# shuaigroup/Renormalizer

Measured on AMD Instinct MI355X. Metric: TDVP-PS sweep site-updates/sec at (Nsite=50, Dbond=256, dphys=2/16), higher is better.
Workload: dtype c128

## Files before the change

### renormalizer_amd/csrc/mpse_contract.hip

```cpp
#include <deque>

#include "mpse_internal.h"
#include "mpse_plans.h"

using namespace mpse_plan;

namespace {

__device__ __forceinline__ long long off2(const mpse_index m, long long i) {
  if (m.lo_ext >= m.ext) return i * m.s_lo;
  const long long hi = i / m.lo_ext;
  return hi * m.s_hi + (i - hi * m.lo_ext) * m.s_lo;
}

template <typename T>
__global__ __launch_bounds__(256) void k_copy_strided(T* dst, const T* src, mpse_index mi, mpse_index ni, mpse_index mo,
                                                      mpse_index no, const int* skip) {
  if (skip && *skip) return;
  const long long nn = ni.ext;
  const long long total = mi.ext * nn;
  const long long stride = (long long)gridDim.x * blockDim.x;
  for (long long t = (long long)blockIdx.x * blockDim.x + threadIdx.x; t < total; t += stride) {
    const long long i = t / nn, j = t - i * nn;
    dst[off2(mo, i) + off2(no, j)] = src[off2(mi, i) + off2(ni, j)];
// ... 376 lines not shown
            o.seg[q].bm = fb + sg.bm_kt0;
          } else if (sg.bm_kind == BM_CENTRE && cm) {
            o.seg[q].bm = cm;
            gd.bm_pitch = cm_pitch;
          }
        }
      }
      gd.masks_stable = stable;
      if (gd.ngrp == 1 && s.groups[0].split2) {
        if (!bufs[B_OUT2]) return mpse_fail(ctx, MPSE_ERR_ARG, "plan: missing second result");
        gd.split2 = true;
        gd.c2 = const_cast<void*>(bufs[B_OUT2]);
      }
      const bool completes =
          &s == &p.steps.back() && gd.ngrp == 1 && s.groups[0].cbuf == B_OUT && s.groups[0].c_off == 0;
      MPSE_TRY(gemm_grouped(ctx, gd, sc, completes ? dot : nullptr));
      continue;
    }
    const char* a = (const char*)bufs[s.a] + size_t(s.a_off) * dtype_size(s.dta);
    const char* b = (const char*)bufs[s.b] + size_t(s.b_off) * dtype_size(s.dtb);
    const int dtc = (s.dta == MPSE_C128 || s.dtb == MPSE_C128) ? MPSE_C128 : MPSE_F64;
    if (dtc != dtype)
      return mpse_fail(ctx, MPSE_ERR_ARG, "plan step dtype mismatch (got %d want %d)", dtc, dtype);
    char* c = (char*)const_cast<void*>(bufs[s.c]) + size_t(s.c_off) * dtype_size(dtc);
    if (!bufs[s.a] || !bufs[s.b] || !bufs[s.c]) return mpse_fail(ctx, MPSE_ERR_ARG, "plan: missing buffer");
    if (s.kind == K_COPY) {
      MPSE_TRY(copy_call(ctx, dtc, a, c, s.ma, s.ka, s.mc, s.nc, skip));
      continue;
    }
    ProductReq rq;
    if (&s == &p.steps.back() && s.c == B_OUT && s.c_off == 0 && s.batch == 1) rq.dot = dot;
// ... 235 lines not shown
```

### renormalizer_amd/csrc/mpse_gemm.hip

```cpp
#include <cstdlib>

#include "mpse_device.h"
#include "mpse_internal.h"
#include "mpse_plans.h"

typedef double v4d __attribute__((ext_vector_type(4)));

static unsigned long long* gemm_trace_ptr(const mpse_ctx* ctx) {
  static const bool f0_only = [] {
    const char* e = getenv("MPSE_GEMM_TRACE_ONLY");
    return e && e[0] == 'f';
  }();
  return (ctx->prof_on && !f0_only) ? ctx->gemm_trace : nullptr;
}

namespace {

struct IdxMap {
  long long s_hi, s_lo;
  int ext, lo;
};

constexpr int GMAX_GRP = 8, GMAX_SEG = 4, GMAX_MIX = 8;
struct GMix {
// ... 10 lines not shown
  GSeg seg[GMAX_SEG];
  double* C;
  int nseg;
  int use_beta;
};
struct GemmGroups {
  GGrp g[GMAX_GRP];
  int ngrp, tiles_m_grp, nkt_seg, am_pitch, bm_pitch;
  int split2, cpd;
  double* C2;
  const unsigned long long* flags;
  int nmix, mix_grp, mix_d, mix_wr;
  long long mix_ld;
  const double* mix_w;
  GMix mix[GMAX_MIX];
};

struct GemmArgs {
  const double* A;
  const double* B;
  double* C;
  IdxMap mA, kA, kB, nB, mC, nC;
  long long sbA, sbB, sbC;
  int M, N, K;
  int tiles_m, tiles_n;
  int mtiles_m, mtiles_n;
  int a_kfast, b_kfast;
  int conjA, conjB;
  int use_beta;
  double alpha_re, alpha_im, beta_re, beta_im;
// ... 18 lines not shown
};


__device__ __forceinline__ void dot_acc(double& re, double& im, double2 c, double2 y) {
  re += c.x * y.x + c.y * y.y;
  im += c.x * y.y - c.y * y.x;
}

__device__ __forceinline__ long long idx_off(const IdxMap& m, int i) {
  if (m.lo == 0x7fffffff) return (long long)i * m.s_lo;
  const int hi = i / m.lo;
  const int l = i - hi * m.lo;
  return (long long)hi * m.s_hi + (long long)l * m.s_lo;
}

#ifndef MPSE_GEMM_3M
#define MPSE_GEMM_3M 1
#endif
constexpr int BM = 64, BN = 64, BK = 16, LDK = BK + 1;

template <bool CA, bool CB, bool KS, int WS, int WI = 2, bool GRP = false>
__global__ __launch_bounds__(64 * WS * WS * (2 / WI), WS == 1 ? 1 : WI == 1 ? 4 : ((CA && CB) ? 2 : 3)) void k_gemm(const GemmArgs g) {
  static_assert(!GRP || (KS && WS == 2), "grouped launches use the single-level 64 x 64 kernel");
  constexpr int TBM = 32 * WS, TBN = 32 * WS, NT = 64 * WS * WS * (2 / WI);
  static_assert(WI == 2 || (WI == 1 && WS == 2), "eight-wave form only for 64 x 64 tiles");
  constexpr int LD = WS == 2 ? 80 : 48;
  constexpr int NLD = TBM * BK / NT;
  constexpr bool CC = CA || CB;
  constexpr int EA = CA ? 2 : 1, EB = CB ? 2 : 1, EC = CC ? 2 : 1;
  __shared__ double smem[(2 + (CA ? 1 : 0) + (CB ? 1 : 0)) * BK * LD];
// ... 25 lines not shown
        half = q & 1;
        t = ((q >> 1) << 3) | (bid & 7);
      } else {
        half = bid & 1;
        t = bid >> 1;
      }
      bs = half;
    }
  }
  if (g.slice_fast) {
    t = bid / g.ksplit;
    bs = bid - t * g.ksplit;
  }
  const int b = bs / g.ksplit;
  const int ks_id = bs - b * g.ksplit;
  if (g.perm) t = g.perm[(ks_id & 1) ? ntile - 1 - t : t];
  int tm = t / g.tiles_n;
  int tn = t - tm * g.tiles_n;
  if (g.die_group == 1) {
    const int x = t & 7, j = t >> 3;
    tm = x + 8 * (j / g.tiles_n);
    tn = j % g.tiles_n;
  } else if (g.die_group == 2) {
    const int x = t & 7, j = t >> 3;
    tn = x + 8 * (j / g.tiles_m);
    tm = j % g.tiles_m;
  }
  if (g.skew && !g.perm && !g.die_group) tn = (tn + tm) % g.tiles_n;

  int grp = 0;
  if constexpr (GRP) {
    grp = tm / g.gg.tiles_m_grp;
    tm -= grp * g.gg.tiles_m_grp;
// ... 466 lines not shown
    for (int kk = 0; kk < BK / 4; ++kk) {
      const int cb = kk & 1;
      if (kk + 1 < BK / 4) read_frag(cb ^ 1, kk + 1);
      mfma_group(cb);
    }
  }
  }

  if (g.trace) tr3 = __builtin_readcyclecounter();
  struct TraceEnd {
    const GemmArgs& g;
    unsigned long long t0, rt0, &t1, &t2, &t3;
    int tid;
    int& ktd;
    __device__ ~TraceEnd() {
      if (g.trace && tid == 0) {
        const unsigned long long slot = atomicAdd(g.trace, 1ull);
        if (slot < GEMM_TRACE_CAP) {
          unsigned long long* r = g.trace + 1 + slot * GEMM_TRACE_WORDS;
          unsigned xcc = 0;
          r[0] = ((unsigned long long)gridDim.x << 32) | (unsigned long long)blockIdx.x;
          r[1] = ((unsigned long long)(CA ? 1 : 0) << 62) | ((unsigned long long)(CB ? 1 : 0) << 61) |
                 ((unsigned long long)g.ksplit << 40) | ((unsigned long long)(unsigned)g.K << 8) | xcc;
          const unsigned hw = __builtin_amdgcn_s_getreg((31 << 11) | 4), xc = __builtin_amdgcn_s_getreg((31 << 11) | 20);
          r[2] = (unsigned long long)(unsigned)ktd | ((unsigned long long)(((xc & 0xf) << 16) | (hw & 0xffff)) << 32);
          r[3] = t0;
          r[4] = t1;
          r[5] = t2;
          r[6] = t3;
          r[7] = __builtin_readcyclecounter();
          r[8] = rt0;
          r[9] = __builtin_amdgcn_s_memrealtime();
        }
      }
    }
  } trace_end{g, tr0, rt0, tr1, tr2, tr3, tid, kt_done};
  if (g.kt_counter && tid == 0 && kt_done) atomicAdd(g.kt_counter, (unsigned long long)kt_done);
  if constexpr (M3) {
#pragma unroll
    for (int i = 0; i < WI; ++i)
#pragma unroll
      for (int j = 0; j < 2; ++j) {
        acc_im[i][j] = acc_im[i][j] - acc_re[i][j] - acc_t2[i][j];
        acc_re[i][j] = acc_re[i][j] - acc_t2[i][j];
      }
  }
  if (g.ksplit > 1) {
    double* wsb = g.ws + (long long)bs * g.M * g.N * EC;
#pragma unroll
// ... 85 lines not shown
            const double* pin = g.Cin ? g.Cin + (idx_off(g.mCin, gi) + cinn) * EC : C + co * EC;
            if constexpr (CC)
              pre_c[i][j][r] = *reinterpret_cast<const double2*>(pin);
            else
              pre_c[i][j][r] = make_double2(*pin, 0.0);
          }
          if (need_y) {
            if constexpr (CC)
              pre_y[i][j][r] = reinterpret_cast<const double2*>(g.dot_y)[co];
            else
              pre_y[i][j][r] = make_double2(g.dot_y[co], 0.0);
          }
        }
    }
  }
#pragma unroll
  for (int j = 0; j < 2; ++j) {
    const int gj = tn * TBN + wn * 32 + j * 16 + (lane & 15);
    if (gj >= g.N) continue;
    const long long coffn = idx_off(g.nC, gj);
#pragma unroll
    for (int i = 0; i < WI; ++i) {
#pragma unroll
      for (int r = 0; r < 4; ++r) {
        const int gi = tm * TBM + wm * WROWS + i * 16 + (lane >> 4) + 4 * r;
        if (gi >= g.M) continue;
        const long long co = idx_off(g.mC, gi) + coffn;
        double* p = C + co * EC;
        const double xr = acc_re[i][j][r];
        if constexpr (CC) {
          const double xi = acc_im[i][j][r];
          double2 o;
          o.x = g.alpha_re * xr - g.alpha_im * xi;
          o.y = g.alpha_re * xi + g.alpha_im * xr;
// ... 9 lines not shown
          *reinterpret_cast<double2*>(p) = o;
          if (need_y) {
            if constexpr (PRE)
              dot_acc(dre, dim, o, pre_y[i][j][r]);
            else
              dot_acc(dre, dim, o, reinterpret_cast<const double2*>(g.dot_y)[co]);
          }
        } else {
          double o = g.alpha_re * xr;
          if (need_c) o += g.beta_re * (g.Cin ? g.Cin[idx_off(g.mCin, gi) + idx_off(g.nCin, gj)] : *p);
          *p = o;
          if (need_y) dre += o * g.dot_y[co];
        }
      }
    }
  }
  if constexpr (WS == 2) {
    if (g.dot_y) {
      __shared__ double s_dot[2 * (NT / 64)];
      dre = wave_sum(dre);
      dim = wave_sum(dim);
      if (lane == 0) {
        s_dot[2 * wave] = dre;
        s_dot[2 * wave + 1] = dim;
      }
      __syncthreads();
      dre = dim = 0.0;
#pragma unroll
      for (int w = 0; w < NT / 64; ++w) {
        dre += s_dot[2 * w];
// ... 20 lines not shown
          key[hi] = a;
        }
      }
      __syncthreads();
    }
}
__device__ __forceinline__ int pow2_at_least(int x) {
  int n = 2;
  while (n < x) n <<= 1;
  return n;
}
__global__ __launch_bounds__(1024) void k_tile_order(const unsigned long long* __restrict__ amask,
                                                       const unsigned long long* __restrict__ bmask, int nkw, int nkt,
                                                       int tiles_m, int tiles_n, int by_die, int* __restrict__ perm,
                                                       const int* __restrict__ skip, const GemmGroups gg,
                                                       unsigned char* __restrict__ flags_out, int flags_pitch) {
  if (skip && *skip) return;
  __shared__ unsigned key[2048], ckey[2048];
  __shared__ int colw[2048];
  __shared__ unsigned char die_of[2048];
  const int ntile = tiles_m * tiles_n, tid = threadIdx.x;
  const bool part = by_die && tiles_n % 8 == 0 && tiles_n <= 2048;
  for (int c = tid; c < 2048; c += 1024) colw[c] = 0;
  __syncthreads();
  for (int i = tid; i < 2048; i += 1024) {
    unsigned cnt = 0;
    if (i < ntile) {
      const int tm = i / tiles_n, tn = i - tm * tiles_n;
      if (gg.ngrp > 0) {
        const int grp = tm / gg.tiles_m_grp, tml = tm - grp * gg.tiles_m_grp;
        const GGrp& G = gg.g[grp];
        for (int q = 0; q < G.nseg; ++q)
          for (int l = 0; l < gg.nkt_seg; ++l) {
            unsigned v = 1;
            if (G.seg[q].am) v &= G.seg[q].am[(long long)tml * gg.am_pitch + l];
            if (G.seg[q].bm) v &= G.seg[q].bm[(long long)tn * gg.bm_pitch + l];
            cnt += v;
            if (flags_out) flags_out[(long long)i * flags_pitch + q * gg.nkt_seg + l] = (unsigned char)v;
          }
        if (flags_out)
          for (int l = G.nseg * gg.nkt_seg; l < flags_pitch; ++l) flags_out[(long long)i * flags_pitch + l] = 0;
      } else {
        for (int w = 0; w < nkw; ++w) {
          unsigned long long x = 0x0101010101010101ull;
          if (amask) x &= amask[(long long)tm * nkw + w];
          if (bmask) x &= bmask[(long long)tn * nkw + w];
          const int valid = nkt - 8 * w;
          if (valid < 8) x &= (1ull << (8 * valid)) - 1ull;
          cnt += __popcll(x);
// ... 15 lines not shown
    __syncthreads();
  }
  for (int i = tid; i < 2048; i += 1024) {
    unsigned k = 0;
    if (i < ntile) {
      const unsigned die = part ? die_of[i % tiles_n] : 0u;
      k = (die << 28) | (key[i] << 16) | (unsigned)(0xFFFF - i);
    }
    key[i] = k;
  }
  __syncthreads();
  bitonic_desc(key, tid, pow2_at_least(ntile));
  const int per_die = ntile / 8;
  for (int i = tid; i < ntile; i += 1024) {
    const int s = part ? (7 - (i & 7)) * per_die + (i >> 3) : i;
    perm[i] = 0xFFFF - (int)(key[s] & 0xFFFFu);
  }
}

template <bool CC>
__global__ __launch_bounds__(256) void k_splitk_reduce(const GemmArgs g, int batch) {
  constexpr int EC = CC ? 2 : 1;
  if (g.skip && *g.skip) return;
  const long long mn = (long long)g.M * g.N;
  const int rows = g.M * batch;
  double dre = 0.0, dim = 0.0;
  for (int row = blockIdx.y; row < rows; row += gridDim.y) {
    const int b = row / g.M;
    const int i = row - b * g.M;
    const double* wrow = g.ws + ((long long)b * g.ksplit * mn + (long long)i * g.N) * EC;
    double* crow = g.C + ((long long)b * g.sbC + idx_off(g.mC, i)) * EC;
// ... 408 lines not shown
      const dim3 og((p.nkt + 3) / 4, oa.tiles > ob.tiles ? oa.tiles : ob.tiles, (unsigned)(2 * d->batch));
      hipLaunchKernelGGL(k_tile_occ, og, dim3(256), 0, ctx->stream, oa, ob, g.K, g.nkw, (int)d->batch, g.skip);
    }
    g.amask = static_cast<const unsigned long long*>(ma.mask);
    g.bmask = static_cast<const unsigned long long*>(mb.mask);
  }

  if (p.order) {
    SolveScope* const keep = sc && sc->keeps_env_masks && ma.stable && mb.stable ? sc : nullptr;
    int* pp = nullptr;
    bool sort = false;
    MPSE_TRY(perm_source(ctx, keep, {g.amask, g.bmask, g.tiles_m, g.tiles_n, p.nkt, nullptr},
                         size_t(g.tiles_m) * g.tiles_n * sizeof(int), PERM, &pp, &sort));
    if (sort)
      hipLaunchKernelGGL(k_tile_order, dim3(1), dim3(1024), 0, ctx->stream, g.amask, g.bmask, g.nkw, p.nkt, g.tiles_m,
                         g.tiles_n, 1, pp, g.skip, GemmGroups(), (unsigned char*)nullptr, 0);
    g.perm = pp;
  }

  count_paths(ctx->gemm_paths, p, d->batch > 1);
  const bool reduce = g.ksplit > 1 && !p.leave_slices;
  launch_gemm(ctx, g, p.nwg, ca, cb, p.fast, p.wide, false, reduce ? dim3((unsigned)p.rgx, (unsigned)p.rgy) : dim3(0),
              (int)d->batch);
  if (prof_this) prof_end(ctx, rec);
  MPSE_HIP(ctx, hipGetLastError());
  return MPSE_OK;
}

int occ_mask_get(mpse_ctx* ctx, SolveScope* sc, const void* ptr, int dtype, mpse_index r, mpse_index k,
                 TmpBuf& tmp, const unsigned char** flags, int* pitch, bool* stable) {
  IdxMap rm, km;
// ... 6 lines not shown
  MPSE_TRY(occ_mask_source(ctx, keep, key, nullptr, tmp.p, &m));
  if (m.scan) {
    const OccOperand oa = occ_operand(key, rm, km, fastest(km) <= fastest(rm), m);
    OccOperand ob = oa;
    ob.tiles = 0;
    hipLaunchKernelGGL(k_tile_occ, dim3(((key.K + BK - 1) / BK + 3) / 4, key.tiles, 2), dim3(256), 0, ctx->stream, oa, ob,
                       key.K, key.nkw, 1, sc ? sc->skip : nullptr);
    MPSE_HIP(ctx, hipGetLastError());
  }
  *flags = static_cast<const unsigned char*>(m.mask);
  *pitch = key.nkw * 8;
  *stable = m.stable;
  return MPSE_OK;
}

static double mix_sources(const GroupedDesc& d) {
  int n = 0;
  for (int t = 0; t < d.nmix; ++t) {
    bool seen = false;
    for (int u = 0; u < t; ++u) seen = seen || d.mix[u].src == d.mix[t].src;
    n += seen ? 0 : 1;
  }
  return n > 1 ? double(n - 1) : 0.0;
}

int gemm_grouped(mpse_ctx* ctx, const GroupedDesc& d, SolveScope* sc, MatvecReq::Dot* dot) {
  GemmArgs g = {};
  if (d.ngrp < 1 || d.ngrp > GMAX_GRP) return mpse_fail(ctx, MPSE_ERR_ARG, "grouped product: 1 .. %d groups", GMAX_GRP);
  if (!fill_maps(g, d.ma, d.ka, d.kb, d.nb, d.mc, d.nc))
    return mpse_fail(ctx, MPSE_ERR_SHAPE, "grouped product: extent out of range");
  if (g.M != g.mC.ext || g.N != g.nC.ext || g.K != g.kB.ext) return mpse_fail(ctx, MPSE_ERR_SHAPE, "grouped product: extents disagree");
  if (g.M == 0 || g.N == 0) return MPSE_OK;
  const bool ca = d.dta == MPSE_C128, cb = d.dtb == MPSE_C128;
  if (!is_single(g.kA) || !is_single(g.kB) || !fast_ok(g, ca, cb) || g.K % BK != 0 || g.K < BK ||
      (d.ngrp > 1 && g.M % BM != 0) || !cb)
    return mpse_fail(ctx, MPSE_ERR_SHAPE, "grouped product: needs single-level K indices, K a multiple of %d, group "
                     "heights a multiple of %d and a complex second operand", BK, BM);
  if (d.split2 && (d.ngrp != 1 || !d.c2 || g.M % BM != 0))
    return mpse_fail(ctx, MPSE_ERR_ARG, "grouped product: halved tiles need one group, whole tile rows and a second result");
  g.alpha_re = 1.0, g.beta_re = 1.0;
  g.ksplit = 1;
// ... 29 lines not shown
  g.use_beta = any_beta;
  if (d.nmix > 0) {
    if (!ca || d.nmix > GMAX_MIX || d.mix_grp < 0 || d.mix_grp >= d.ngrp || d.grp[d.mix_grp].beta != 1.0 || !d.mix_w ||
        d.mix_d < 1 || BM % d.mix_d != 0 || g.M % BM != 0 || d.mix_wr < 1 || d.mix_ld < g.N)
      return mpse_fail(ctx, MPSE_ERR_ARG, "grouped product: bad epilogue mix");
    gg.nmix = d.nmix, gg.mix_grp = d.mix_grp, gg.mix_d = d.mix_d, gg.mix_wr = d.mix_wr, gg.mix_ld = d.mix_ld;
    gg.mix_w = static_cast<const double*>(d.mix_w);
    for (int t = 0; t < d.nmix; ++t) {
      if (!d.mix[t].src || d.mix[t].delta <= -d.mix_d || d.mix[t].delta >= d.mix_d)
        return mpse_fail(ctx, MPSE_ERR_ARG, "grouped product: bad epilogue mix term");
      gg.mix[t] = GMix{static_cast<const double*>(d.mix[t].src), d.mix[t].b, d.mix[t].f, d.mix[t].delta, 0};
    }
  }

  const int nkt_max = max_seg * gg.nkt_seg;
  const mpse_plan::GroupedPlan p = mpse_plan::grouped_plan(g.M, g.N, d.ngrp, nkt_max, any_mask, d.split2, ca, n_cu_of(ctx));
  const long long ntile = (long long)p.tiles_m * p.tiles_n;
  if (ntile > 0x7fffffffLL) return mpse_fail(ctx, MPSE_ERR_SHAPE, "grouped product: grid too large");
  g.tiles_m = p.tiles_m;
  g.nkw = p.nkw;
  g.die_group = p.die_group;
  if (dot && d.ngrp == 1 && p.nwg >= 1 && p.nwg <= dot->cap) {
    g.dot_y = static_cast<const double*>(dot->y);
    g.dot_part = dot->part;
    dot->nb_out = (int)p.nwg;
  }
  mpse_ctx::ProfRec rec;
  const int variant = (ca ? 1 : 0) + (cb ? 2 : 0);
  const double mnk = double(g.M) * double(g.N) * double(g.K) * segs;
  const bool prof_this = prof_begin(ctx, variant, mnk * ((ca && cb) ? 8.0 : 4.0),
                                    segs * (double(g.M) * g.K * (ca ? 16 : 8) + double(g.K) * g.N * 16.0) +
                                        double(d.ngrp) * double(g.M) * g.N * 16.0 * (any_beta ? 2 : 1) +
                                        mix_sources(d) * double(g.M) * g.N * 16.0,
                                    &rec);
  g.kt_counter = prof_this && ctx->prof_ktiles ? ctx->prof_ktiles + variant : nullptr;

  TmpBuf PERM(ctx);
  if (p.order) {
    const size_t perm_bytes = (size_t(ntile) * sizeof(int) + 7) & ~size_t(7), flag_pitch = size_t(g.nkw) * 8;
    int* pp = nullptr;
    bool sort = false;
    MPSE_TRY(perm_source(ctx, sc && sc->keeps_env_masks && d.masks_stable ? sc : nullptr,
                         {gg.g[0].seg[0].am, gg.g[0].seg[0].bm, g.tiles_m, g.tiles_n, nkt_max + 1000 * d.ngrp, nullptr},
                         perm_bytes + size_t(ntile) * flag_pitch, PERM, &pp, &sort));
    if (sort)
      hipLaunchKernelGGL(k_tile_order, dim3(1), dim3(1024), 0, ctx->stream, (const unsigned long long*)nullptr,
                         (const unsigned long long*)nullptr, 0, nkt_max, g.tiles_m, g.tiles_n, d.split2 ? 0 : 1, pp,
                         g.skip, gg, reinterpret_cast<unsigned char*>(pp) + perm_bytes, (int)flag_pitch);
    g.perm = pp;
    g.gg.flags = reinterpret_cast<const unsigned long long*>(reinterpret_cast<const char*>(pp) + perm_bytes);
  }

  count_paths(ctx->gemm_paths, d);
  launch_gemm(ctx, g, p.nwg, ca, cb, true, p.wide, true);
  if (prof_this) prof_end(ctx, rec);
  MPSE_HIP(ctx, hipGetLastError());
  return MPSE_OK;
}

extern "C" int mpse_gemm(mpse_ctx* ctx, const mpse_gemm_desc* d, const void* A, const void* B, void* C) {
  if (ctx && d && MPSE_RECORDING(ctx)) {
    const mpse_gemm_desc dc = *d;
    ctx->defer_ops[ctx->defer_recording].push_back([ctx, dc, A, B, C] { return mpse_gemm(ctx, &dc, A, B, C); });
    return MPSE_OK;
  }
  return gemm_impl(ctx, d, A, B, C, d ? (d->skip_zero_tiles & 3) : 0, nullptr, nullptr);
}

extern "C" int mpse_gemm_path_stats(mpse_ctx* ctx, int64_t* counts, int n) {
// ... 50 lines not shown
```

### renormalizer_amd/csrc/mpse_internal.h

```cpp
#pragma once
#include <hip/hip_runtime.h>

#include <cstdarg>
#include <cstdlib>
#include <cstdint>
#include <cstdio>
#include <cstring>
#include <functional>
#include <map>
#include <memory>
#include <mutex>
#include <string>
#include <unordered_map>
#include <vector>

#include "../../include/mpsengine.h"

struct mpse_ctx {
  int device = 0;
  hipStream_t stream = nullptr;
  int n_cu = 0;
  char err[512] = {0};
  char dev_name[128] = {0};

// ... 53 lines not shown
  std::unordered_map<const void*, WSiteEntry> wsite_info;
  std::vector<std::function<int()>> defer_ops[2];
  int defer_recording = -1;
  int defer_armed = -1;
  bool defer_hold = false;
  std::vector<void*> defer_frees;
  struct CMask {
    const void* ptr = nullptr;
    long long bytes = 0;
  } cmask_pending;
  unsigned long long* gemm_trace = nullptr;
  bool gemm_trace_checked = false;
  long long f0_launches[2] = {0, 0};
  enum GemmPath {
    GP_LAUNCH, GP_GENERAL, GP_WIDE, GP_SPLIT_B1, GP_SPLIT_BN, GP_DIE1, GP_DIE2, GP_SKEW, GP_ORDER, GP_MASK,
    GP_MASK_GLOBAL, GP_GROUPED, GP_GROUPED_SPLIT2, GP_GROUPED_MIX, GP_WMIX, GP_COUNT
  };
  long long gemm_paths[GP_COUNT] = {0};
  long long qr_chol_calls = 0, qr_chol_fallbacks = 0, qr_calls = 0;
  bool qr_optimistic = false;
  int qr_scheme = -1;
  int* qr_words_dev = nullptr;
  long long lz_batch_members = 0, lz_batch_single = 0;
  enum LzPath {
    LP_SYNC, LP_ASYNC_DONE, LP_HOST_FIRST, LP_HOST_LATER, LP_LIMIT, LP_BD_ASYNC, LP_BD_SYNC, LP_FULL, LP_CONV,
    LP_NOCONV, LP_MERGED, LP_WAITS, LP_GROW, LP_PARTS, LP_VMASK, LP_UNVEC, LP_RESCALE, LP_ALIAS_RESTART, LP_COUNT
  };
  long long lz_paths[LP_COUNT] = {0};
  enum PcgStat {
    PS_SOLVES, PS_ITERS, PS_MATVECS, PS_WAITS, PS_END_TOL, PS_END_MAXITER, PS_END_CURVATURE, PS_TWOLAYER, PS_MASKED,
    PS_COUNT
// ... 175 lines not shown
struct MatvecReq {
  struct Dot {
    const void* y = nullptr;
    double* part = nullptr;
    int cap = 0;
    int nb_out = 0;
  } dot;
  struct Parts {
    void* ptr = nullptr;
    long long cap_elems = 0, n = 0;
    int used = 0;
    bool masked_ok = false;
    const unsigned long long* mask = nullptr;
    int mask_row = 0, mask_tiles = 0;
  } parts;
};

struct ProductReq {
  MatvecReq::Dot* dot = nullptr;
  const void* cin = nullptr;
  mpse_index cin_m{}, cin_n{};
  void* slices = nullptr;
  size_t slices_cap = 0;
  int slices_used = 0;
};

int heff_apply(mpse_ctx* ctx, int dtype, const mpse_heff* h, const void* C, void* out, SolveScope* sc,
               MatvecReq* mv);
int heff_apply2(mpse_ctx* ctx, int dtype, const mpse_heff* h, const void* C, void* out, SolveScope* sc);
int heff_apply_ft(mpse_ctx* ctx, int dtype, const mpse_heff_ft* h, const void* C, void* out, SolveScope* sc);
// ... 74 lines not shown
struct GroupedDesc {
  int dta = MPSE_F64, dtb = MPSE_F64;
  mpse_index ma{}, ka{}, kb{}, nb{}, mc{}, nc{};
  int ngrp = 0;
  GroupedGrp grp[8];
  int am_pitch = 0, bm_pitch = 0;
  bool masks_stable = false;
  bool split2 = false;
  void* c2 = nullptr;
  int nmix = 0, mix_grp = 0;
  GroupedMixTerm mix[8];
  const void* mix_w = nullptr;
  int mix_d = 0, mix_wr = 0;
  long long mix_ld = 0;
};
int gemm_grouped(mpse_ctx* ctx, const GroupedDesc& d, SolveScope* sc, MatvecReq::Dot* dot);
int occ_mask_get(mpse_ctx* ctx, SolveScope* sc, const void* ptr, int dtype, mpse_index r, mpse_index k,
                 TmpBuf& tmp, const unsigned char** flags, int* pitch, bool* stable);

int publish_and_wait(mpse_ctx* ctx, const double* dsrc, int count, int slot);
int publish_wait_seq(mpse_ctx* ctx, double seq, const double* dsrc, int count, int slot);
struct PublishAt {
  double* pub;
  volatile double* seq_slot;
  double seq;
};
__attribute__((visibility("hidden"))) PublishAt publish_target(mpse_ctx* ctx, bool wait_here, int slot);
__attribute__((visibility("hidden"))) int publish_collect(mpse_ctx* ctx, const PublishAt& at, const void* dsrc, size_t stride,
                                                          int B, int W, int slot, void* host_out);

int dotc_sync(mpse_ctx* ctx, int dtype, const void* x, const void* y, int64_t n, double* re, double* im);
// ... 24 lines not shown
```

### renormalizer_amd/csrc/mpse_lanczos.hip

```cpp
#include <cmath>
#include <complex>
#include <cstdlib>
#include <utility>

#include "mpse_internal.h"
#include "mpse_vec_kernels.h"

namespace {

template <bool VEC>
__global__ __launch_bounds__(RED_THREADS) void k_scale_into_dev(double* dst, const double* __restrict__ src,
                                                                long long n_doubles,
                                                                const double* __restrict__ partial, int nb,
                                                                double* __restrict__ b2_out,
                                                                const int* __restrict__ done) {
  if (done && *done) return;
  double b2, im;
  sum_partials(partial, nb, b2, im);
  if (blockIdx.x == 0 && threadIdx.x == 0) {
    b2_out[0] = b2;
    b2_out[1] = im;
  }
  const double s = 1.0 / sqrt(b2);
  const long long stride = (long long)gridDim.x * blockDim.x;
// ... 714 lines not shown
  int vm_row = 0, vm_kw = 0;
  static const bool vmask_on = [] {
    const char* e = getenv("MPSE_VEC_MASK");
    return !(e && e[0] == '0');
  }();
  if (vmask_on && vec16 && cplx && scope.cmask.ptr && h->dims.Dl_ket > 0 && h->dims.Dl_bra == h->dims.Dl_ket &&
      h->dims.Dr_bra == h->dims.Dr_ket && n < (int64_t(1) << 31)) {
    const int64_t Dl = h->dims.Dl_ket, N = n / Dl;
    const int64_t nkw = ((Dl + 15) / 16 + 7) / 8;
    if (N * Dl == n && N % 64 == 0 && scope.cmask.bytes == (N / 64) * nkw * 8) {
      vmask = static_cast<const unsigned char*>(scope.cmask.ptr);
      vm_row = (int)N;
      vm_kw = (int)(nkw * 8);
    }
  }
  auto dot_partials = [&](const void* x, const void* y, double* dst) {
    ProfScope ps(ctx, 4, 0.0, 2.0 * vbytes);
    MPSE_LAUNCH_TF(ctx, cplx, k_dot_partial, dim3(nb), dim3(RED_THREADS), (const double*)x, (const double*)y, (long long)n,
                   dst, done);
    ps.end();
  };
  double* part_b2[2] = {ctx->dscratch + 4 * RED_MAX_BLOCKS, ctx->dscratch + 8 * RED_MAX_BLOCKS};
  {
    ProfScope ps(ctx, 4, 0.0, 3.0 * vbytes);
    MPSE_LAUNCH_TF(ctx, cplx, k_lz_start, dim3(nb), dim3(RED_THREADS), (double*)vec(0), (const double*)Cin, (long long)n,
                   part_b2[0], ctl);
    ps.end();
  }
  MPSE_HIP(ctx, hipGetLastError());

// ... 8 lines not shown
  };
  bool waited = false;
  LzCtl hc;
  memset(&hc, 0, sizeof(hc));
  for (int j = 0;; ++j) {
    scope.krylov_lo = V.as<char>();
    scope.krylov_hi = V.as<char>() + size_t(cap) * n * es;
    MatvecReq mv;
    mv.dot.y = vec(j);
    mv.dot.part = part_a;
    mv.dot.cap = DOT_CAP;
    mv.parts.ptr = W.p;
    mv.parts.cap_elems = wcap;
    mv.parts.n = n;
    mv.parts.masked_ok = f0_parts > 0 && vec16;
    MPSE_TRY(heff_apply(ctx, dtype, h, vec(j), W.p, &scope, &mv));
    const unsigned long long* pmask = mv.parts.mask;
    const int prow = mv.parts.mask_row, ptiles = mv.parts.mask_tiles;
    const int used = mv.parts.used;
    const int nparts = used > 0 ? used : (used == -2 ? 2 : 1);
    const bool two = nparts > 1;
    const bool dot_done = mv.dot.nb_out > 0;
    const int a_nb = dot_done ? mv.dot.nb_out : nb;
    if (!dot_done) {
      if (two) return mpse_fail(ctx, MPSE_ERR_ARG, "expm_lanczos: a two-part matvec result without its dot partials");
      dot_partials(W.p, vec(j), part_a);
    }
    if (j + 2 > cap) {
      const int ncap = sch.grown();
      ++ctx->lz_paths[mpse_ctx::LP_GROW];
// ... 568 lines not shown
```

### renormalizer_amd/csrc/mpse_plans.h

```cpp
#pragma once
#include <cstdint>
#include <cstdlib>
#include <algorithm>
#include <cstring>
#include <string>
#include <utility>
#include <vector>

#include "../../include/mpsengine.h"

namespace mpse_plan {

enum Buf { B_L = 0, B_R, B_W0, B_W1, B_C, B_BRA, B_OUT, B_T1, B_T2, B_T3, B_W2, B_W3, B_OUT2, B_COUNT };
inline int w_buf(int layer) { return layer == 0 ? B_W0 : layer == 1 ? B_W1 : layer == 2 ? B_W2 : B_W3; }

enum Kind { K_GEMM = 0, K_COPY = 1, K_WMIX = 2, K_GGEMM = 3 };


constexpr int G_MAXGRP = 8, G_MAXSEG = 4, WM_MAXDST = 4, WM_MAXTERM = 4;
constexpr int EPI_MAXTERM = 8, EPI_MAXBAND = 2;

struct WBlock {
  int b, f;
  bool ident;
// ... 1047 lines not shown
      if (cap_y >= 1 && p.rgy > cap_y) p.rgy = cap_y;
      producers = p.rgx * p.rgy;
    }
    if (producers >= 1 && producers <= s.dot_cap) p.dot_producers = producers;
  }
  p.masks = (s.skip_hint & 3) && s.k_single && p.nkt >= 2 && s.batch <= 16384;
  p.nkw = p.masks ? (p.nkt + 7) / 8 : 0;
  p.order = s.batch == 1 && p.masks && order_pays(ntile, ntile * p.ksplit, s.n_cu);
  if (!p.order && p.ksplit == 1 && s.batch == 1)
    p.die_group = die_group_rule(ntile, p.tiles_m, p.tiles_n, double(s.M) * (s.ca ? 2 : 1), double(s.N) * (s.cb ? 2 : 1));
  p.fast = s.k_single && s.fast_ok;
  p.wide = p.fast && p.nwg <= s.n_cu && p.nkt >= 2;
  return p;
}

struct GroupedPlan {
  int tiles_m, tiles_n, nkw, die_group;
  bool order, wide;
  long long nwg;
};
inline GroupedPlan grouped_plan(long long M, long long N, int ngrp, int nkt_max, bool any_mask, bool split2, bool ca,
                                int n_cu) {
  GroupedPlan p{};
  p.tiles_m = int((M + 63) / 64) * ngrp, p.tiles_n = int((N + 63) / 64);
  const long long ntile = (long long)p.tiles_m * p.tiles_n;
  p.nwg = ntile * (split2 ? 2 : 1);
  p.nkw = (any_mask && (nkt_max + 7) / 8 <= 64) ? (nkt_max + 7) / 8 : 0;
  p.order = p.nkw > 0 && order_pays(ntile, ntile, n_cu, split2);
  if (!p.order) p.die_group = die_group_rule(ntile, p.tiles_m, p.tiles_n, double(M) * ngrp * (ca ? 2 : 1), double(N) * 2);
  p.wide = p.nwg <= n_cu;
  return p;
}

}
```

### renormalizer_amd/engine.py

```python
import collections
import ctypes as C
import math
import os
import threading

import numpy as np

_HERE = os.path.dirname(os.path.abspath(__file__))
LIB_PATH = os.environ.get("RENO_MPSENGINE") or os.path.join(_HERE, "csrc", "libmpsengine.so")

F64, C128 = 0, 1
MPSE_OK, MPSE_ERR_OOM, MPSE_ERR_SHAPE, MPSE_ERR_NOCONV, MPSE_ERR_HIP, MPSE_ERR_ARG = 0, 1, 2, 3, 4, 5
DOMAIN_L, DOMAIN_R = 0, 1

STATUS = {0: "OK", 1: "OOM", 2: "SHAPE", 3: "NOCONV", 4: "HIP", 5: "ARG"}


PcgResult = collections.namedtuple("PcgResult", "status iters relres lvalue")


class EngineError(RuntimeError):
    pass


# ... 740 lines not shown
        return a.value, b.value, c.value

    def heff_fused_stats(self):
        a, b = C.c_int64(), C.c_int64()
        self._check(self.lib.mpse_heff_fused_stats(self.ctx, C.byref(a), C.byref(b)))
        return a.value, b.value

    GEMM_PATHS = ("launches", "general", "eight_wave", "split_b1", "split_batched", "die_group1", "die_group2", "skew",
                  "tile_order", "masks", "masks_global", "grouped", "grouped_split2")

    def gemm_path_stats(self):
        return self._stats_dict(self.lib.mpse_gemm_path_stats, self.GEMM_PATHS)

    def wfold_path_stats(self):
        n = len(self.GEMM_PATHS)
        v = (C.c_int64 * (n + 2))()
        self._check(self.lib.mpse_gemm_path_stats(self.ctx, v, n + 2))
        return {"grouped_mix": int(v[n]), "wmix": int(v[n + 1])}

    def block_qr_optimistic(self, on):
        self._check(self.lib.mpse_block_qr_optimistic(self.ctx, int(bool(on))))

    def block_qr_scheme(self, scheme):
        self._check(self.lib.mpse_block_qr_scheme(self.ctx, int(scheme)))

    def block_qr_check(self):
        v = C.c_int(0)
        self._check(self.lib.mpse_block_qr_check(self.ctx, C.byref(v)))
        return bool(v.value)

    def block_qr_pass_stats(self):
        a, b = C.c_int64(0), C.c_int64(0)
        self._check(self.lib.mpse_block_qr_pass_stats(self.ctx, C.byref(a), C.byref(b)))
# ... 119 lines not shown
```

Before: 597.5.

## Skip dead output tiles in grouped GEMM using Lanczos vector occupancy mask

Passes the Krylov vector's block-sparsity mask into the final grouped GEMM of the effective-Hamiltonian apply. The tile-ordering kernel marks output tiles whose rows and columns are all structurally zero as dead and encodes them as negated permutation entries, and those workgroups exit early after zeroing their dot partials. It also adds a cross-wave shared-memory reduction of dot partials for a wide eight-wave split2 launch, and rewrites the profiling byte estimate. The gain depends on how many output tiles are dead, and it adds a more expensive ordering pass plus extra barriers in the epilogue.

```diff
diff --git a/renormalizer_amd/csrc/mpse_contract.hip b/renormalizer_amd/csrc/mpse_contract.hip
--- a/renormalizer_amd/csrc/mpse_contract.hip
+++ b/renormalizer_amd/csrc/mpse_contract.hip
@@ -414,7 +414,8 @@
       }
       const bool completes =
           &s == &p.steps.back() && gd.ngrp == 1 && s.groups[0].cbuf == B_OUT && s.groups[0].c_off == 0;
-      MPSE_TRY(gemm_grouped(ctx, gd, sc, completes ? dot : nullptr));
+      MPSE_TRY(gemm_grouped(ctx, gd, sc, completes ? dot : nullptr,
+                            completes && mv && mv->out_mask.mask ? &mv->out_mask : nullptr));
       continue;
     }
     const char* a = (const char*)bufs[s.a] + size_t(s.a_off) * dtype_size(s.dta);
diff --git a/renormalizer_amd/csrc/mpse_gemm.hip b/renormalizer_amd/csrc/mpse_gemm.hip
--- a/renormalizer_amd/csrc/mpse_gemm.hip
+++ b/renormalizer_amd/csrc/mpse_gemm.hip
@@ -48,6 +48,9 @@
   long long mix_ld;
   const double* mix_w;
   GMix mix[GMAX_MIX];
+  const unsigned char* omask;
+  int om_pitch, om_d;
+  int dot4;
 };
 
 struct GemmArgs {
@@ -96,6 +99,26 @@
   return (long long)hi * m.s_hi + (long long)l * m.s_lo;
 }
 
+__device__ __forceinline__ void trace_record(const GemmArgs& g, bool ca, bool cb, unsigned long long t0,
+                                             unsigned long long rt0, unsigned long long t1, unsigned long long t2,
+                                             unsigned long long t3, int ktd) {
+  const unsigned long long slot = atomicAdd(g.trace, 1ull);
+  if (slot >= GEMM_TRACE_CAP) return;
+  unsigned long long* r = g.trace + 1 + slot * GEMM_TRACE_WORDS;
+  r[0] = ((unsigned long long)gridDim.x << 32) | (unsigned long long)blockIdx.x;
+  r[1] = ((unsigned long long)(ca ? 1 : 0) << 62) | ((unsigned long long)(cb ? 1 : 0) << 61) |
+         ((unsigned long long)g.ksplit << 40) | ((unsigned long long)(unsigned)g.K << 8);
+  const unsigned hw = __builtin_amdgcn_s_getreg((31 << 11) | 4), xc = __builtin_amdgcn_s_getreg((31 << 11) | 20);
+  r[2] = (unsigned long long)(unsigned)ktd | ((unsigned long long)(((xc & 0xf) << 16) | (hw & 0xffff)) << 32);
+  r[3] = t0;
+  r[4] = t1;
+  r[5] = t2;
+  r[6] = t3;
+  r[7] = __builtin_readcyclecounter();
+  r[8] = rt0;
+  r[9] = __builtin_amdgcn_s_memrealtime();
+}
+
 #ifndef MPSE_GEMM_3M
 #define MPSE_GEMM_3M 1
 #endif
@@ -151,9 +174,27 @@
   }
   const int b = bs / g.ksplit;
   const int ks_id = bs - b * g.ksplit;
-  if (g.perm) t = g.perm[(ks_id & 1) ? ntile - 1 - t : t];
+  bool dead = false;
+  if (g.perm) {
+    t = g.perm[(ks_id & 1) ? ntile - 1 - t : t];
+    if constexpr (GRP) {
+      dead = t < 0;
+      t = dead ? ~t : t;
+    }
+  }
   int tm = t / g.tiles_n;
   int tn = t - tm * g.tiles_n;
+  if constexpr (GRP) {
+    if (dead) {
+      if (g.dot_y && tid == 0) {
+        const long long slot = (long long)bs * ntile + t;
+        g.dot_part[2 * slot] = 0.0;
+        g.dot_part[2 * slot + 1] = 0.0;
+      }
+      if (g.trace && tid == 0) trace_record(g, CA, CB, tr0, rt0, tr0, tr0, tr0, 0);
+      return;
+    }
+  }
   if (g.die_group == 1) {
     const int x = t & 7, j = t >> 3;
     tm = x + 8 * (j / g.tiles_n);
@@ -650,25 +691,7 @@
     int tid;
     int& ktd;
     __device__ ~TraceEnd() {
-      if (g.trace && tid == 0) {
-        const unsigned long long slot = atomicAdd(g.trace, 1ull);
-        if (slot < GEMM_TRACE_CAP) {
-          unsigned long long* r = g.trace + 1 + slot * GEMM_TRACE_WORDS;
-          unsigned xcc = 0;
-          r[0] = ((unsigned long long)gridDim.x << 32) | (unsigned long long)blockIdx.x;
-          r[1] = ((unsigned long long)(CA ? 1 : 0) << 62) | ((unsigned long long)(CB ? 1 : 0) << 61) |
-                 ((unsigned long long)g.ksplit << 40) | ((unsigned long long)(unsigned)g.K << 8) | xcc;
-          const unsigned hw = __builtin_amdgcn_s_getreg((31 << 11) | 4), xc = __builtin_amdgcn_s_getreg((31 << 11) | 20);
-          r[2] = (unsigned long long)(unsigned)ktd | ((unsigned long long)(((xc & 0xf) << 16) | (hw & 0xffff)) << 32);
-          r[3] = t0;
-          r[4] = t1;
-          r[5] = t2;
-          r[6] = t3;
-          r[7] = __builtin_readcyclecounter();
-          r[8] = rt0;
-          r[9] = __builtin_amdgcn_s_memrealtime();
-        }
-      }
+      if (g.trace && tid == 0) trace_record(g, CA, CB, t0, rt0, t1, t2, t3, ktd);
     }
   } trace_end{g, tr0, rt0, tr1, tr2, tr3, tid, kt_done};
   if (g.kt_counter && tid == 0 && kt_done) atomicAdd(g.kt_counter, (unsigned long long)kt_done);
@@ -784,10 +807,23 @@
         }
     }
   }
+  constexpr bool HAND = GRP && PRE && WI == 1;
+  bool hand = false;
+  auto hslot = [&]() { return smem + 1024 + (((wm >> 1) * 2 + wn) * 64 + lane) * 2; };
+  if constexpr (HAND) {
+    hand = g.gg.dot4 != 0 && need_y;
+    if (hand) __syncthreads();
+  }
 #pragma unroll
   for (int j = 0; j < 2; ++j) {
     const int gj = tn * TBN + wn * 32 + j * 16 + (lane & 15);
     if (gj >= g.N) continue;
+    if constexpr (HAND) {
+      if (hand) {
+        if (wm & 1) __syncthreads();
+        if ((wm & 1) || j > 0) dre = hslot()[0], dim = hslot()[1];
+      }
+    }
     const long long coffn = idx_off(g.nC, gj);
 #pragma unroll
     for (int i = 0; i < WI; ++i) {
@@ -827,6 +863,20 @@
         }
       }
     }
+    if constexpr (HAND) {
+      if (hand) {
+        if (!((wm & 1) && j == 1)) hslot()[0] = dre, hslot()[1] = dim;
+        if (!(wm & 1)) {
+          __syncthreads();
+          if (j == 0) __syncthreads();
+        } else if (j == 0) {
+          __syncthreads();
+        }
+      }
+    }
+  }
+  if constexpr (HAND) {
+    if (hand && !(wm & 1)) dre = dim = 0.0;
   }
   if constexpr (WS == 2) {
     if (g.dot_y) {
@@ -877,25 +927,29 @@
                                                        const unsigned long long* __restrict__ bmask, int nkw, int nkt,
                                                        int tiles_m, int tiles_n, int by_die, int* __restrict__ perm,
                                                        const int* __restrict__ skip, const GemmGroups gg,
-                                                       unsigned char* __restrict__ flags_out, int flags_pitch) {
+                                                       unsigned char* __restrict__ flags_out, int flags_pitch,
+                                                       int om_M, int om_N) {
   if (skip && *skip) return;
   __shared__ unsigned key[2048], ckey[2048];
   __shared__ int colw[2048];
-  __shared__ unsigned char die_of[2048];
+  __shared__ unsigned char die_of[2048], dead[2048];
   const int ntile = tiles_m * tiles_n, tid = threadIdx.x;
   const bool part = by_die && tiles_n % 8 == 0 && tiles_n <= 2048;
   for (int c = tid; c < 2048; c += 1024) colw[c] = 0;
   __syncthreads();
   for (int i = tid; i < 2048; i += 1024) {
     unsigned cnt = 0;
+    dead[i] = 0;
     if (i < ntile) {
       const int tm = i / tiles_n, tn = i - tm * tiles_n;
       if (gg.ngrp > 0) {
         const int grp = tm / gg.tiles_m_grp, tml = tm - grp * gg.tiles_m_grp;
         const GGrp& G = gg.g[grp];
+        const bool off = gg.omask && !mpse_plan::out_tile_live(gg.omask, gg.om_pitch, gg.om_d, om_N, om_M, tm, tn);
+        dead[i] = off ? 1 : 0;
         for (int q = 0; q < G.nseg; ++q)
           for (int l = 0; l < gg.nkt_seg; ++l) {
-            unsigned v = 1;
+            unsigned v = off ? 0 : 1;
             if (G.seg[q].am) v &= G.seg[q].am[(long long)tml * gg.am_pitch + l];
             if (G.seg[q].bm) v &= G.seg[q].bm[(long long)tn * gg.bm_pitch + l];
             cnt += v;
@@ -941,7 +995,8 @@
   const int per_die = ntile / 8;
   for (int i = tid; i < ntile; i += 1024) {
     const int s = part ? (7 - (i & 7)) * per_die + (i >> 3) : i;
-    perm[i] = 0xFFFF - (int)(key[s] & 0xFFFFu);
+    const int t = 0xFFFF - (int)(key[s] & 0xFFFFu);
+    perm[i] = dead[t] ? ~t : t;
   }
 }
 
@@ -1380,7 +1435,7 @@
                          size_t(g.tiles_m) * g.tiles_n * sizeof(int), PERM, &pp, &sort));
     if (sort)
       hipLaunchKernelGGL(k_tile_order, dim3(1), dim3(1024), 0, ctx->stream, g.amask, g.bmask, g.nkw, p.nkt, g.tiles_m,
-                         g.tiles_n, 1, pp, g.skip, GemmGroups(), (unsigned char*)nullptr, 0);
+                         g.tiles_n, 1, pp, g.skip, GemmGroups(), (unsigned char*)nullptr, 0, 0, 0);
     g.perm = pp;
   }
 
@@ -1417,17 +1472,35 @@
   return MPSE_OK;
 }
 
-static double mix_sources(const GroupedDesc& d) {
-  int n = 0;
-  for (int t = 0; t < d.nmix; ++t) {
-    bool seen = false;
-    for (int u = 0; u < t; ++u) seen = seen || d.mix[u].src == d.mix[t].src;
-    n += seen ? 0 : 1;
-  }
-  return n > 1 ? double(n - 1) : 0.0;
-}
-
-int gemm_grouped(mpse_ctx* ctx, const GroupedDesc& d, SolveScope* sc, MatvecReq::Dot* dot) {
+static double grouped_bytes(const GroupedDesc& d, double M, double N, double K, bool ca) {
+  const void* seen[3][GMAX_GRP * GMAX_SEG + GMAX_MIX];
+  int n[3] = {0, 0, 0};
+  auto fresh = [&](int w, const void* p) {
+    for (int i = 0; i < n[w]; ++i)
+      if (seen[w][i] == p) return false;
+    seen[w][n[w]++] = p;
+    return true;
+  };
+  double bytes = 0.0, betas = 0.0;
+  for (int i = 0; i < d.ngrp; ++i) {
+    for (int q = 0; q < d.grp[i].nseg; ++q) {
+      if (fresh(0, d.grp[i].seg[q].A)) bytes += M * K * (ca ? 16.0 : 8.0);
+      if (fresh(1, d.grp[i].seg[q].B)) bytes += K * N * 16.0;
+    }
+    bytes += M * N * 16.0;
+    betas += d.grp[i].beta != 0.0 ? 1.0 : 0.0;
+  }
+  if (d.nmix > 0) {
+    betas -= 1.0;
+    const int w = (K == N && ca) ? 0 : 2;
+    for (int t = 0; t < d.nmix; ++t)
+      if (fresh(w, d.mix[t].src)) bytes += M * N * 16.0;
+  }
+  return bytes + betas * M * N * 16.0;
+}
+
+int gemm_grouped(mpse_ctx* ctx, const GroupedDesc& d, SolveScope* sc, MatvecReq::Dot* dot,
+                 const MatvecReq::OutMask* om) {
   GemmArgs g = {};
   if (d.ngrp < 1 || d.ngrp > GMAX_GRP) return mpse_fail(ctx, MPSE_ERR_ARG, "grouped product: 1 .. %d groups", GMAX_GRP);
   if (!fill_maps(g, d.ma, d.ka, d.kb, d.nb, d.mc, d.nc))
@@ -1487,7 +1560,12 @@
   }
 
   const int nkt_max = max_seg * gg.nkt_seg;
-  const mpse_plan::GroupedPlan p = mpse_plan::grouped_plan(g.M, g.N, d.ngrp, nkt_max, any_mask, d.split2, ca, n_cu_of(ctx));
+  const long long nwg_all = (long long)((g.M + BM - 1) / BM) * g.tiles_n * (d.split2 ? 2 : 1);
+  const int om_d = om && om->mask && om->row > 0 && om->row % g.N == 0 ? om->row / g.N : 0;
+  const bool om_fits = om_d > 0 && d.ngrp == 1 && dot && nwg_all <= dot->cap && g.M % om_d == 0 &&
+                       (g.M / om_d + 15) / 16 <= om->pitch && om->row % 64 == 0;
+  const mpse_plan::GroupedPlan p =
+      mpse_plan::grouped_plan(g.M, g.N, d.ngrp, nkt_max, any_mask, d.split2, ca, n_cu_of(ctx), om_fits);
   const long long ntile = (long long)p.tiles_m * p.tiles_n;
   if (ntile > 0x7fffffffLL) return mpse_fail(ctx, MPSE_ERR_SHAPE, "grouped product: grid too large");
   g.tiles_m = p.tiles_m;
@@ -1498,13 +1576,13 @@
     g.dot_part = dot->part;
     dot->nb_out = (int)p.nwg;
   }
+  const bool out_mask = om_fits && p.order && g.dot_y;
+  if (out_mask) gg.omask = om->mask, gg.om_pitch = om->pitch, gg.om_d = om_d;
   mpse_ctx::ProfRec rec;
   const int variant = (ca ? 1 : 0) + (cb ? 2 : 0);
   const double mnk = double(g.M) * double(g.N) * double(g.K) * segs;
   const bool prof_this = prof_begin(ctx, variant, mnk * ((ca && cb) ? 8.0 : 4.0),
-                                    segs * (double(g.M) * g.K * (ca ? 16 : 8) + double(g.K) * g.N * 16.0) +
-                                        double(d.ngrp) * double(g.M) * g.N * 16.0 * (any_beta ? 2 : 1) +
-                                        mix_sources(d) * double(g.M) * g.N * 16.0,
+                                    grouped_bytes(d, double(g.M), double(g.N), double(g.K), ca),
                                     &rec);
   g.kt_counter = prof_this && ctx->prof_ktiles ? ctx->prof_ktiles + variant : nullptr;
 
@@ -1514,18 +1592,22 @@
     int* pp = nullptr;
     bool sort = false;
     MPSE_TRY(perm_source(ctx, sc && sc->keeps_env_masks && d.masks_stable ? sc : nullptr,
-                         {gg.g[0].seg[0].am, gg.g[0].seg[0].bm, g.tiles_m, g.tiles_n, nkt_max + 1000 * d.ngrp, nullptr},
+                         {gg.g[0].seg[0].am, gg.g[0].seg[0].bm, g.tiles_m, g.tiles_n,
+                          nkt_max + 1000 * d.ngrp + (out_mask ? 1000000 : 0), nullptr},
                          perm_bytes + size_t(ntile) * flag_pitch, PERM, &pp, &sort));
     if (sort)
       hipLaunchKernelGGL(k_tile_order, dim3(1), dim3(1024), 0, ctx->stream, (const unsigned long long*)nullptr,
                          (const unsigned long long*)nullptr, 0, nkt_max, g.tiles_m, g.tiles_n, d.split2 ? 0 : 1, pp,
-                         g.skip, gg, reinterpret_cast<unsigned char*>(pp) + perm_bytes, (int)flag_pitch);
+                         g.skip, gg, reinterpret_cast<unsigned char*>(pp) + perm_bytes, (int)flag_pitch, g.M, g.N);
     g.perm = pp;
     g.gg.flags = reinterpret_cast<const unsigned long long*>(reinterpret_cast<const char*>(pp) + perm_bytes);
   }
 
   count_paths(ctx->gemm_paths, d);
-  launch_gemm(ctx, g, p.nwg, ca, cb, true, p.wide, true);
+  ctx->gemm_paths[mpse_ctx::GP_GROUPED_OUTMASK] += out_mask;
+  const bool om_wide = out_mask && d.split2 && ca && !p.wide && g.N % BN == 0;
+  gg.dot4 = om_wide ? 1 : 0;
+  launch_gemm(ctx, g, p.nwg, ca, cb, true, p.wide || om_wide, true);
   if (prof_this) prof_end(ctx, rec);
   MPSE_HIP(ctx, hipGetLastError());
   return MPSE_OK;
diff --git a/renormalizer_amd/csrc/mpse_internal.h b/renormalizer_amd/csrc/mpse_internal.h
--- a/renormalizer_amd/csrc/mpse_internal.h
+++ b/renormalizer_amd/csrc/mpse_internal.h
@@ -91,7 +91,7 @@
   long long f0_launches[2] = {0, 0};
   enum GemmPath {
     GP_LAUNCH, GP_GENERAL, GP_WIDE, GP_SPLIT_B1, GP_SPLIT_BN, GP_DIE1, GP_DIE2, GP_SKEW, GP_ORDER, GP_MASK,
-    GP_MASK_GLOBAL, GP_GROUPED, GP_GROUPED_SPLIT2, GP_GROUPED_MIX, GP_WMIX, GP_COUNT
+    GP_MASK_GLOBAL, GP_GROUPED, GP_GROUPED_SPLIT2, GP_GROUPED_MIX, GP_WMIX, GP_GROUPED_OUTMASK, GP_COUNT
   };
   long long gemm_paths[GP_COUNT] = {0};
   long long qr_chol_calls = 0, qr_chol_fallbacks = 0, qr_calls = 0;
@@ -297,6 +297,10 @@
     const unsigned long long* mask = nullptr;
     int mask_row = 0, mask_tiles = 0;
   } parts;
+  struct OutMask {
+    const unsigned char* mask = nullptr;
+    int row = 0, pitch = 0;
+  } out_mask;
 };
 
 struct ProductReq {
@@ -401,7 +405,8 @@
   int mix_d = 0, mix_wr = 0;
   long long mix_ld = 0;
 };
-int gemm_grouped(mpse_ctx* ctx, const GroupedDesc& d, SolveScope* sc, MatvecReq::Dot* dot);
+int gemm_grouped(mpse_ctx* ctx, const GroupedDesc& d, SolveScope* sc, MatvecReq::Dot* dot,
+                 const MatvecReq::OutMask* om = nullptr);
 int occ_mask_get(mpse_ctx* ctx, SolveScope* sc, const void* ptr, int dtype, mpse_index r, mpse_index k,
                  TmpBuf& tmp, const unsigned char** flags, int* pitch, bool* stable);
 
diff --git a/renormalizer_amd/csrc/mpse_lanczos.hip b/renormalizer_amd/csrc/mpse_lanczos.hip
--- a/renormalizer_amd/csrc/mpse_lanczos.hip
+++ b/renormalizer_amd/csrc/mpse_lanczos.hip
@@ -752,6 +752,10 @@
       vm_kw = (int)(nkw * 8);
     }
   }
+  static const bool omask_on = [] {
+    const char* e = getenv("MPSE_OUT_MASK");
+    return !(e && e[0] == '0');
+  }();
   auto dot_partials = [&](const void* x, const void* y, double* dst) {
     ProfScope ps(ctx, 4, 0.0, 2.0 * vbytes);
     MPSE_LAUNCH_TF(ctx, cplx, k_dot_partial, dim3(nb), dim3(RED_THREADS), (const double*)x, (const double*)y, (long long)n,
@@ -790,6 +794,7 @@
     mv.parts.cap_elems = wcap;
     mv.parts.n = n;
     mv.parts.masked_ok = f0_parts > 0 && vec16;
+    if (vmask && omask_on) mv.out_mask.mask = vmask, mv.out_mask.row = vm_row, mv.out_mask.pitch = vm_kw;
     MPSE_TRY(heff_apply(ctx, dtype, h, vec(j), W.p, &scope, &mv));
     const unsigned long long* pmask = mv.parts.mask;
     const int prow = mv.parts.mask_row, ptiles = mv.parts.mask_tiles;
diff --git a/renormalizer_amd/csrc/mpse_plans.h b/renormalizer_amd/csrc/mpse_plans.h
--- a/renormalizer_amd/csrc/mpse_plans.h
+++ b/renormalizer_amd/csrc/mpse_plans.h
@@ -1085,19 +1085,32 @@
   return p;
 }
 
+#if defined(__HIPCC__)
+__host__ __device__
+#endif
+inline bool out_tile_live(const unsigned char* mask, int pitch, int d, int Dr, int M, int tm, int tn) {
+  const int r1 = 64 * tm + 64 < M ? 64 * tm + 64 : M, l0 = 64 * tn, l1 = 64 * tn + 63 < Dr - 1 ? 64 * tn + 63 : Dr - 1;
+  for (int r = 64 * tm; r < r1; ++r) {
+    const int a = r / d, sg = r - a * d;
+    for (int ct = (sg * Dr + l0) >> 6; ct <= (sg * Dr + l1) >> 6; ++ct)
+      if (mask[(long long)ct * pitch + (a >> 4)]) return true;
+  }
+  return false;
+}
+
 struct GroupedPlan {
   int tiles_m, tiles_n, nkw, die_group;
   bool order, wide;
   long long nwg;
 };
 inline GroupedPlan grouped_plan(long long M, long long N, int ngrp, int nkt_max, bool any_mask, bool split2, bool ca,
-                                int n_cu) {
+                                int n_cu, bool out_mask = false) {
   GroupedPlan p{};
   p.tiles_m = int((M + 63) / 64) * ngrp, p.tiles_n = int((N + 63) / 64);
   const long long ntile = (long long)p.tiles_m * p.tiles_n;
   p.nwg = ntile * (split2 ? 2 : 1);
   p.nkw = (any_mask && (nkt_max + 7) / 8 <= 64) ? (nkt_max + 7) / 8 : 0;
-  p.order = p.nkw > 0 && order_pays(ntile, ntile, n_cu, split2);
+  p.order = p.nkw > 0 && order_pays(ntile, ntile, n_cu, split2 || out_mask);
   if (!p.order) p.die_group = die_group_rule(ntile, p.tiles_m, p.tiles_n, double(M) * ngrp * (ca ? 2 : 1), double(N) * 2);
   p.wide = p.nwg <= n_cu;
   return p;
diff --git a/renormalizer_amd/engine.py b/renormalizer_amd/engine.py
--- a/renormalizer_amd/engine.py
+++ b/renormalizer_amd/engine.py
@@ -778,9 +778,9 @@
 
     def wfold_path_stats(self):
         n = len(self.GEMM_PATHS)
-        v = (C.c_int64 * (n + 2))()
-        self._check(self.lib.mpse_gemm_path_stats(self.ctx, v, n + 2))
-        return {"grouped_mix": int(v[n]), "wmix": int(v[n + 1])}
+        v = (C.c_int64 * (n + 3))()
+        self._check(self.lib.mpse_gemm_path_stats(self.ctx, v, n + 3))
+        return {"grouped_mix": int(v[n]), "wmix": int(v[n + 1]), "grouped_outmask": int(v[n + 2])}
 
     def block_qr_optimistic(self, on):
         self._check(self.lib.mpse_block_qr_optimistic(self.ctx, int(bool(on))))
```

Result: faster. 608.6, median of 6 (+1.9%).
